# martinhoT/Footsies-Gym

Hardware: AMD Instinct MI355X
Metric: env-steps/sec (whole node) at 65 536 envs; bit-exact vs Unity ref (higher is better)
Workload: dtype int32+f32 (reward f64); 1 GPU; C3: 65536 arenas/GPU, self-play random actions, P2 external, auto-reset same-step; envs_per_gpu=65536, global_envs=65536, mode=fused, ticks_per_launch=1000, trajectory=packed records (fs_step_n_packed), parallelism=arena-shard x1, action_rows=2665, action_rows_needed=2665, action_rows_repeat=False

## Files before the change

footsies_gym_amd/csrc/fs_kernels.hip:

```cpp
#include <hip/hip_runtime.h>

#include <cstdio>

#include "fs_internal.h"
#include "fs_tables.h"
#include "fs_policy.h"

#pragma clang fp contract(off)

namespace fsk {

constexpr int NONE = 31;
constexpr uint32_t IN_LEFT = 1, IN_RIGHT = 2, IN_ATTACK = 4;

__shared__ Tables sT;
__shared__ ParserTable sParser;

constexpr int kBlock = 256;

template <bool G>
__device__ __forceinline__ const Tables& tabs() {
  if constexpr (G) return kTables;
  else return sT;
}
constexpr int kTabLds = 0, kTabGlobal = 1;


typedef float F2 __attribute__((ext_vector_type(2)));
__device__ __forceinline__ F2 splat(float v) { return F2{v, v}; }

struct Fighter {
  float x;
  uint32_t hist;
  int act, frame, stun, vital, guard, hits, buf, rsv, hold;
  uint32_t in_back, prox, won;
  int rec;
  float px, ux0, ux1, hx0, hx1;
  float pw, phw;
  uint32_t flip;
  float y;
  float py, uy0, uy1, hy0, hy1;
};

constexpr uint32_t kHdrRecCountMask = 0x7fff;
constexpr int kHdrRec1 = 15, kHdrRec2 = 18, kHdrAct1 = 21, kHdrAct2 = 24;
constexpr int kHdrPending = 27, kHdrHasTerm = 28, kHdrP2Bot = 29;
struct Header {
  uint32_t rec_count;
  uint32_t rec[2], act[2];
  uint32_t pending, has_term;
  uint32_t p2bot;
};
__device__ __forceinline__ Header unpack_header(uint32_t h) {
  return Header{h & kHdrRecCountMask, {(h >> kHdrRec1) & 7, (h >> kHdrRec2) & 7},
                {(h >> kHdrAct1) & 7, (h >> kHdrAct2) & 7}, (h >> kHdrPending) & 1, (h >> kHdrHasTerm) & 1,
                (h >> kHdrP2Bot) & 1};
}
__device__ __forceinline__ uint32_t pack_header(const Header& H) {
  return H.rec_count | (H.rec[0] << kHdrRec1) | (H.rec[1] << kHdrRec2) | (H.act[0] << kHdrAct1) |
         (H.act[1] << kHdrAct2) | (H.pending << kHdrPending) | (H.has_term << kHdrHasTerm) | (H.p2bot << kHdrP2Bot);
}

struct Arena {
  Fighter f0, f1;
  int frame_count;
  Header h;
  double cum;
  uint4 rng;
  uint2 bw[2];
// ... 93 lines not shown
  x &= 0x55555555u;
  x = (x | (x >> 1)) & 0x33333333u;
  x = (x | (x >> 2)) & 0x0F0F0F0Fu;
  x = (x | (x >> 4)) & 0x00FF00FFu;
  x = (x | (x >> 8)) & 0x0000FFFFu;
  return x;
}
__device__ __forceinline__ uint32_t spread_even(uint32_t x) {
  x &= 0x0000FFFFu;
  x = (x | (x << 8)) & 0x00FF00FFu;
  x = (x | (x << 4)) & 0x0F0F0F0Fu;
  x = (x | (x << 2)) & 0x33333333u;
  x = (x | (x << 1)) & 0x55555555u;
  return x;
}
__device__ __forceinline__ uint32_t split_hist(uint32_t raw, int k) {
  const uint32_t rel = k == 0 ? raw : (((raw & 0x55555555u) << 1) | ((raw >> 1) & 0x55555555u));
  return compact_even(rel) | (compact_even(rel >> 1) << 16);
}
__device__ __forceinline__ uint32_t raw_hist(uint32_t h, int k) {
  const uint32_t b = spread_even(h), f = spread_even(h >> 16);
  return k == 0 ? (b | (f << 1)) : (f | (b << 1));
}

constexpr uint32_t kRelLut0 = 0xE4E4u, kRelLut1 = 0xD8D8u;

__device__ __forceinline__ InputEval update_input(Fighter& f, uint32_t in, uint32_t rlut) {
  const uint32_t old_hist = f.hist;
  const int old_hold = f.hold;
  const uint32_t r0 = __builtin_amdgcn_ubfe(rlut, in << 1, 2);
  f.hist = ((old_hist << 1) & 0xFFFEFFFEu) | (r0 & 1) | ((r0 & 2) << 15);
  f.hold = (in & IN_ATTACK) ? min(old_hold + 1, 63) : 0;
  InputEval e;
  e.held = r0;
  const uint32_t atk_now = (in >> 2) & 1u;
  const uint32_t held_long = ((uint32_t)(old_hold - (kSpecialHoldFrame - 1)) >> 31) ^ 1u;
  const uint32_t was_up = (uint32_t)(old_hold - 1) >> 31;
  e.atk = (held_long & ~atk_now & 1u) | ((atk_now & was_up) << 1);
  const uint32_t B = old_hist & 0xFFFFu, F = old_hist >> 16, E = B | F;
  const uint32_t win = (1u << (kDashAllowFrame - 1)) - 1u;
  const uint32_t j = (uint32_t)__builtin_ctz((E & win) | (1u << (kDashAllowFrame - 1)));
  const uint32_t neutral = min((~E >> (j + 1)) & win, 1u);
  const uint32_t isF = ((F & win) >> j) & 1u, isB = ((B & win) >> j) & 1u;
  const uint32_t fd = isF & ~isB & neutral & (r0 >> 1) & ~F;
  const uint32_t bd = isB & ~isF & neutral & r0 & ~B;
  e.dash = (fd & 1u) | ((bd & 1u) << 1);
  return e;
}

#ifndef FS_PARSER_TABLE
#define FS_PARSER_TABLE 1
#endif
constexpr bool kParserTable = FS_PARSER_TABLE != 0;
constexpr uint32_t kRelLut4_0 = 0x64206420u, kRelLut4_1 = 0x62406240u;
__device__ __forceinline__ uint32_t pairs_hist(uint32_t h) { return spread_even(h) | (spread_even(h >> 16) << 1); }
__device__ __forceinline__ uint32_t unpair_hist(uint32_t p) { return compact_even(p) | (compact_even(p >> 1) << 16); }
__device__ __forceinline__ uint32_t parser_state_row(uint32_t h) {
  constexpr uint32_t w = kDashAllowFrame - 1, cap = kParserRunCap;
  static_assert(cap == w + 1 && 2 * w <= 16 && kParserStates == w * 3 * cap + 1, "the automaton of gen_tables.py");
  const uint32_t B = h & 0xFFFFu, F = h >> 16, E = B | F;
  const uint32_t j = (uint32_t)__builtin_ctz((E & ((1u << w) - 1u)) | (1u << w));
  const uint32_t kind = ((B >> j) & 1u) | (((F >> j) & 1u) << 1);
  const uint32_t run = min((uint32_t)__builtin_ctz(~(E >> j)), cap);
  const uint32_t s = j == w ? 0u : ((run - 1u) * w + j) * 3u + kind;
  return s << 3;
}
__device__ __forceinline__ uint32_t parser_read_row(uint32_t row, uint32_t rowb, uint32_t rlut4) {
  const uint32_t r0x2 = __builtin_amdgcn_ubfe(rlut4, rowb << 2, 3);
  return *reinterpret_cast<const uint16_t*>(reinterpret_cast<const char*>(&sParser.next[0][0]) + (row | r0x2));
}
__device__ __forceinline__ InputEval take_input(Fighter& f, uint32_t in, uint32_t pe) {
  const int old_hold = f.hold;
  InputEval e;
  e.held = (pe >> 1) & 3u;
  e.dh = pe & 0x1Eu;
  e.dash = (pe >> 3) & 3u;
  f.hist = (f.hist << 2) | e.held;
  f.hold = (in & IN_ATTACK) ? min(old_hold + 1, 63) : 0;
  const uint32_t atk_now = (in >> 2) & 1u;
  const uint32_t held_long = ((uint32_t)(old_hold - (kSpecialHoldFrame - 1)) >> 31) ^ 1u;
  const uint32_t was_up = (uint32_t)(old_hold - 1) >> 31;
  e.atk = (held_long & ~atk_now & 1u) | ((atk_now & was_up) << 1);
  return e;
}

__device__ __forceinline__ void set_action(Fighter& f, int a) {
  f.act = a;
  f.frame = 0;
  f.hits = 0;
  f.buf = NONE;
  f.rsv = NONE;
}

typedef uint32_t AInfo __attribute__((ext_vector_type(4)));
template <bool G>
__device__ __forceinline__ AInfo action_info(int a) { return reinterpret_cast<const AInfo*>(tabs<G>().action)[a]; }
__device__ __forceinline__ AInfo stand_info() {
  AInfo i;
  i.x = kStandInfo[0];
  i.y = kStandInfo[1];
  i.z = kStandInfo[2];
  i.w = kStandInfo[3];
  return i;
}
__device__ __forceinline__ int ai_frame_count(AInfo i) { return (int)(int16_t)(i.x & 0xffffu); }
__device__ __forceinline__ int ai_loop_from(AInfo i) { return (int)(int16_t)(i.x >> 16); }
__device__ __forceinline__ bool ai_always_cancel(AInfo i) { return (i.y & 0xffu) != 0; }
__device__ __forceinline__ int ai_cancel_lo(AInfo i) { return (int)((i.y >> 16) & 0xffu); }
__device__ __forceinline__ int ai_cancel_hi(AInfo i) { return (int)(i.y >> 24); }
__device__ __forceinline__ uint32_t ai_cancel_mask(AInfo i) { return i.z; }
static_assert(sizeof(ActionInfo) == 16, "ActionInfo must be 16 bytes");

__device__ __forceinline__ void increment_action_frame(Fighter& f, AInfo ai) {
  const bool stunned = f.stun > 0;
  f.stun -= stunned ? 1 : 0;
  const int next = f.frame + 1;
  const int loop_from = ai_loop_from(ai);
  const int looped = (next >= ai_frame_count(ai) && loop_from >= 0) ? loop_from : next;
  f.frame = stunned ? f.frame : looped;
}

template <bool INV = false>
__device__ __forceinline__ uint32_t request_sel_cls(const Fighter& f, const InputEval& e, uint32_t cls, bool& keep) {
  const int rsv = f.rsv, buf = f.buf;
  const bool has_rsv = rsv != NONE;
  const bool won = f.won != 0;
  const bool early = (f.stun <= 0) & (has_rsv | ((buf != NONE) & (kCanCancelOnWhiff | (f.hits > 0))));
  const int a0 = has_rsv ? rsv : buf;
  const uint32_t in8 = ((9u * cls + 3u * e.atk + e.dash) << 3) | (e.held << 1) | (uint32_t)f.prox;
  const uint32_t idx = ((uint32_t)f.act << 8) | (in8 ^ (uint32_t)f.act);
  if constexpr (INV) {
    keep = early;
    if constexpr (kParserTable) {
      const uint32_t t8 = (((9u * cls + 3u * e.atk) << 3) + e.dh) | (uint32_t)f.prox;
      return early ? (uint32_t)(kReqEarly + a0) : (((uint32_t)f.act << 8) | (t8 ^ (uint32_t)f.act));
    }
    return early ? (uint32_t)(kReqEarly + a0) : idx;
  }
  keep = early | won;
  return won ? (uint32_t)kReqWin + 3u * (uint32_t)f.act + cls : (early ? (uint32_t)(kReqEarly + a0) : idx);
}
__device__ __forceinline__ uint32_t request_cls(const Fighter& f, AInfo ai) {
  const bool ended = f.frame >= ai_frame_count(ai);
  const bool inwin = (f.frame >= ai_cancel_lo(ai)) & (f.frame <= ai_cancel_hi(ai));
  return ended ? 2u : (inwin ? 1u : 0u);
}
__device__ __forceinline__ uint32_t request_sel(const Fighter& f, const InputEval& e, AInfo ai, bool& keep) {
  return request_sel_cls(f, e, request_cls(f, ai), keep);
}
__device__ __forceinline__ bool apply_request(Fighter& f, uint32_t q, bool keep, const InputEval& e, uint32_t* rec) {
  const bool set = ((q >> 11) & 1u) != 0;
  const bool bset = ((q >> 10) & 1u) != 0;
  f.act = set ? (int)(q & 31u) : f.act;
  f.buf = set ? NONE : (bset ? (int)((q >> 5) & 31u) : f.buf);
  f.frame = set ? 0 : f.frame;
  f.hits = set ? 0 : f.hits;
  f.rsv = set ? NONE : f.rsv;
  f.in_back = keep ? f.in_back : (e.held & 1u);
  f.prox = keep ? f.prox : 0u;
  *rec = (q >> 12) & 255u;
  return set;
}
template <bool G>
__device__ __forceinline__ bool update_action_request(Fighter& f, const InputEval& e, AInfo ai, uint32_t* rec) {
  bool keep;
  const uint32_t sel = request_sel(f, e, ai, keep);
  return apply_request(f, tabs<G>().req_table[sel], keep, e, rec);
}

template <int FM>
__device__ __forceinline__ void update_movement(Fighter& f, float v) {
  float nx;
  if constexpr (FM == FS_FLOAT_DOUBLE) nx = (float)__dadd_rn((double)f.x, __dmul_rn((double)v, (double)kDt));
  else nx = __fadd_rn(f.x, __fmul_rn(v, kDt));
  f.x = (f.stun <= 0 && v != 0.0f) ? nx : f.x;
}

typedef float F4 __attribute__((ext_vector_type(4)));
typedef uint32_t U4 __attribute__((ext_vector_type(4)));
struct RecGeo {
  F4 push;
  F4 hurt;
  F4 hit;
};
template <bool G>
__device__ __forceinline__ RecGeo frame_rec(uint32_t k, uint32_t rec) {
  const Tables& T = tabs<G>();
// ... 213 lines not shown
  switch (b) {
    case 0: return r <= 3 ? AP_NONE : AP_DELAY_SPECIAL;
    case 1: return r <= 1 ? AP_NONE : r <= 3 ? AP_ONE_HIT : AP_DELAY_SPECIAL;
    case 2: return r == 0 ? AP_NONE : r == 1 ? AP_ONE_HIT : AP_TWO_HIT;
    case 3: return r <= 1 ? AP_ONE_HIT : r <= 3 ? AP_TWO_HIT : r == 4 ? AP_IMMEDIATE_SPECIAL : AP_DELAY_SPECIAL;
    default: return r == 0 ? AP_ONE_HIT : AP_TWO_HIT;
  }
}
__device__ __forceinline__ bool attack_forced(uint32_t b, uint32_t opp) {
  constexpr uint32_t kAny = (1u << A_DAMAGE) | (1u << A_GUARD_BREAK) | (1u << A_N_SPECIAL) | (1u << A_B_SPECIAL);
  constexpr uint32_t kMid = (1u << A_N_ATTACK) | (1u << A_B_ATTACK);
  return (((b == 1 ? kAny | kMid : kAny) >> opp) & 1u) != 0;
}

struct alignas(16) BotDraw {
  uint32_t map;
  uint32_t magic;
  uint32_t n;
  uint32_t c16;
};
struct alignas(16) BotTables {
  BotDraw draw[2][5];
  uint32_t codes[2][8][8];
  uint8_t len[2][8];
};
constexpr BotDraw make_draw(uint32_t n, uint32_t map) {
  return BotDraw{map, (uint32_t)(((1u << 23) + n - 1) / n), n, 65536u % n};
}
constexpr BotTables make_bot_tables() {
  BotTables t{};
  for (int b = 0; b < 5; b++) {
    uint32_t mm = 0, ma = 0;
    for (uint32_t r = 0; r < move_draw_n(b); r++) mm |= move_draw_plan(b, r) << (4 * r);
    for (uint32_t r = 0; r < attack_draw_n(b); r++) ma |= attack_draw_plan(b, r) << (4 * r);
    t.draw[1][b] = make_draw(move_draw_n(b), mm);
    t.draw[0][b] = make_draw(attack_draw_n(b), ma);
  }
  for (uint32_t p = 0; p < 7; p++) {
    t.len[1][p] = (uint8_t)move_plan_len(p);
    for (uint32_t i = 0; i < move_plan_len(p); i++) t.codes[1][p][i >> 4] |= move_plan_input(p, i) << (2 * (i & 15));
  }
  for (uint32_t p = 0; p < 5; p++) {
    t.len[0][p] = (uint8_t)attack_plan_len(p);
    for (uint32_t i = 0; i < attack_plan_len(p); i++)
      t.codes[0][p][i >> 4] |= (uint32_t)((i < attack_plan_hold(p)) | ((p == AP_TWO_HIT) & (i == 4))) << (2 * (i & 15));
  }
  return t;
}
static_assert(move_plan_len(MP_FAR1) <= 8 * 16 && attack_plan_len(AP_DELAY_SPECIAL) <= 8 * 16,
              "plans fit eight code words");
__constant__ const BotTables kBot = make_bot_tables();
__shared__ BotTables sBot;
static_assert(sizeof(Tables) + sizeof(BotTables) <= 40 * 1024, "the staged tables: at most 40 KB per block");
static_assert(sizeof(Tables) + sizeof(ParserTable) <= 40 * 1024, "(no kernel stages both: see step_body)");
template <bool G>
__device__ __forceinline__ const BotTables& bots() {
  if constexpr (G) return kBot;
  else return sBot;
}

typedef __attribute__((address_space(1))) void* GlobalPtr;
typedef __attribute__((address_space(3))) void* LdsPtr;
template <int BYTES>
__device__ __forceinline__ void lds_dma_copy(void* dst, const void* src) {
  static_assert(BYTES % 16 == 0, "16-byte pieces");
  constexpr int kChunks = BYTES / 16, kPieces = (kChunks + 63) / 64;
  const int wave = threadIdx.x >> 6, lane = threadIdx.x & 63;
  for (int j = wave; j < kPieces; j += kBlock / 64) {
    const int c = j * 64 + lane;
    if (c < kChunks)
      __builtin_amdgcn_global_load_lds((GlobalPtr)(reinterpret_cast<const char*>(src) + c * 16),
                                       (LdsPtr)(reinterpret_cast<char*>(dst) + j * 1024), 16, 0, 0);
  }
}
template <bool BOTS = true, bool PARSER = false>
__device__ __forceinline__ void stage_tables() {
  static_assert(!(BOTS && PARSER), "the bot kernels have no specialised loop");
  lds_dma_copy<sizeof(Tables)>(&sT, &kTables);
  if constexpr (BOTS) lds_dma_copy<sizeof(BotTables)>(&sBot, &kBot);
  if constexpr (PARSER) lds_dma_copy<sizeof(ParserTable)>(&sParser, &kParser);
  __syncthreads();
}

__device__ __forceinline__ uint32_t draw_mod(uint32_t x, const BotDraw& d) {
  const uint32_t v = __umul24(x >> 16, d.c16) + (x & 0xFFFFu);
  const uint64_t prod = (uint64_t)(v & 0xFFFFFFu) * (uint64_t)(d.magic & 0xFFFFFFu);
  const uint32_t q = (uint32_t)(prod >> 23);
  return v - __umul24(d.n, q);
}

struct Bot {
  uint4 rng;
  uint32_t plan, idx;
  uint32_t prev_opp;
  float prev_dist;
};

template <int FM>
__device__ __forceinline__ float bot_distance(float x1, float x2) {
  return fabsf(fsub<FM>(x2, x1));
}

__device__ __forceinline__ uint32_t xpair(uint32_t v);
struct BotPre {
  uint32_t code_word;
  BotDraw w;
  uint32_t len;
};
__device__ __forceinline__ uint32_t bot_bucket(float d) {
  return d > 4.0f ? 0u : d > 3.0f ? 1u : d > 2.5f ? 2u : d > 2.0f ? 3u : 4u;
}
template <bool G>
__device__ __forceinline__ BotPre bot_prefetch(const Bot& b, uint32_t q) {
  const uint32_t p = b.plan != 0 ? b.plan - 1 : 0u;
  BotPre r;
  r.code_word = bots<G>().codes[q][p][b.idx >> 4];
  r.w = bots<G>().draw[q][bot_bucket(b.prev_dist)];
  r.len = bots<G>().len[q][p];
  return r;
}

template <bool G>
__device__ __forceinline__ uint32_t bot_next_input(Bot& b, uint32_t q, float dist, uint32_t opp_act, const BotPre& pre) {
  const float d = b.prev_dist;
  const uint32_t opp = b.prev_opp;
  b.prev_dist = dist;
  b.prev_opp = opp_act;
  const uint32_t bucket = bot_bucket(d);
  const bool busy = b.plan != 0;
  const uint32_t i = b.idx;
  const uint32_t code = (pre.code_word >> (2 * (i & 15))) & 3u;
  const uint32_t mine = busy ? (q ? code : code << 2) : 0u;
  const bool o_busy = xpair((uint32_t)busy) != 0;
// ... 68 lines not shown
  }
  if (b.aplan != 0) {
    const uint32_t p = b.aplan - 1, i = b.aidx;
    in |= ((bots<G>().codes[0][p][i >> 4] >> (2 * (i & 15))) & 1u) << 2;
    b.aidx = i + 1;
    if (b.aidx == bots<G>().len[0][p]) b.aplan = 0;
  } else if (attack_forced(bucket, opp)) {
    b.aplan = AP_TWO_HIT + 1;
    b.aidx = 0;
  } else {
    const BotDraw w = bots<G>().draw[0][bucket];
    b.aplan = ((w.map >> (4 * draw_mod(rng_next(rng), w))) & 15u) + 1;
    b.aidx = 0;
  }
  return in;
}

__device__ __forceinline__ void bot_full_reset(FullBot& b, float dist, uint32_t opp_act) {
  b.mplan = b.midx = b.aplan = b.aidx = 0;
  b.prev_dist = dist;
  b.prev_opp = opp_act;
  b.ready = true;
}

__device__ __forceinline__ uint32_t xpair(uint32_t v) {
  return (uint32_t)__builtin_amdgcn_mov_dpp((int)v, 0xB1 , 0xF, 0xF, true);
}
__device__ __forceinline__ int xpair(int v) { return (int)xpair((uint32_t)v); }
__device__ __forceinline__ float xpair(float v) { return __uint_as_float(xpair(__float_as_uint(v))); }
__device__ __forceinline__ uint32_t xp1(uint32_t v) {
  return (uint32_t)__builtin_amdgcn_mov_dpp((int)v, 0xA0 , 0xF, 0xF, true);
}
__device__ __forceinline__ uint32_t xp2(uint32_t v) {
  return (uint32_t)__builtin_amdgcn_mov_dpp((int)v, 0xF5 , 0xF, 0xF, true);
}
__device__ __forceinline__ float xp1(float v) { return __uint_as_float(xp1(__float_as_uint(v))); }
__device__ __forceinline__ float xp2(float v) { return __uint_as_float(xp2(__float_as_uint(v))); }

struct Lane {
  Fighter f;
  uint32_t k;
  int frame_count;
  uint32_t rec_count;
  uint32_t pending, has_term;
  double cum;
  uint32_t rec;
  uint32_t act;
  uint32_t bin;
  uint32_t p2bot;
  AInfo ai;
  uint32_t te;
  uint32_t pe;
  uint32_t ps;
  Bot bot;
  FullBot fb;
  uint4 rng;
};

template <int V>
__device__ __forceinline__ void load_lane(Lane& L, const DevState& s, int a, uint32_t k) {
  const int l = 2 * a + (int)k;
  L.k = k;
  L.f.x = reinterpret_cast<const float*>(s.pos)[l];
  L.f.hist = reinterpret_cast<const uint32_t*>(s.hist)[l];
  const uint2 w = reinterpret_cast<const uint2*>(s.fpk)[l];
  const int2 aw = s.aw[a];
  L.cum = s.cum[a];
  unpack_fighter(L.f, w.x, w.y);
  const uint32_t h = (uint32_t)aw.y;
  L.frame_count = aw.x;
  L.rec_count = h & kHdrRecCountMask;
  L.rec = (h >> (k ? kHdrRec2 : kHdrRec1)) & 7;
  L.act = (h >> (k ? kHdrAct2 : kHdrAct1)) & 7;
  L.pending = (h >> kHdrPending) & 1;
  L.has_term = (h >> kHdrHasTerm) & 1;
  L.p2bot = (h >> kHdrP2Bot) & 1;
  L.bin = 0;
  if constexpr (V == FS_P2_BOT) {
    L.bot.rng = s.rng[a];
    const uint2 b = s.bot[a];
    L.bot.plan = k ? ((b.x >> kBotMoveQueue) & 7) : ((b.x >> kBotAtkQueue) & 7);
    L.bot.idx = k ? ((b.x >> kBotMoveIdx) & 127) : ((b.x >> kBotAtkIdx) & 127);
    L.bot.prev_opp = (b.x >> kBotPrevOpp) & 31;
    L.bot.prev_dist = __uint_as_float(b.y);
    L.bin = (b.x >> kBotInput) & 7;
  } else if constexpr (V == kActors) {
    L.rng = s.rng[a];
    L.fb = unpack_bot(k ? s.bot[a] : s.bot1[a], L.bin);
  }
}

template <int V>
__device__ __forceinline__ void store_lane(const Lane& L, const DevState& s, int a) {
  const int l = 2 * a + (int)L.k;
  const uint64_t w = pack_fighter(L.f);
  reinterpret_cast<float*>(s.pos)[l] = L.f.x;
  reinterpret_cast<uint32_t*>(s.hist)[l] = L.f.hist;
  reinterpret_cast<uint2*>(s.fpk)[l] = make_uint2((uint32_t)w, (uint32_t)(w >> 32));
  const uint32_t other = xpair(L.rec | (L.act << 3));
  if (L.k == 0) {
    const uint32_t p2bot = V == FS_P2_BOT ? 1u : V == kActors ? (uint32_t)L.p2bot : 0u;
    const uint32_t h = L.rec_count | (L.rec << kHdrRec1) | ((other & 7) << kHdrRec2) | (L.act << kHdrAct1) |
                       ((other >> 3) << kHdrAct2) | ((uint32_t)L.pending << kHdrPending) |
                       ((uint32_t)L.has_term << kHdrHasTerm) | (p2bot << kHdrP2Bot);
    s.aw[a] = make_int2(L.frame_count, (int)h);
    s.cum[a] = L.cum;
// ... 277 lines not shown
  const PkRec v = packed_record(L, 0u);
  const uint32_t ox = xpair(v.x), oz = xpair(v.z);
  RecQ q;
  if (L.k == 0) {
    q.x = __builtin_amdgcn_perm(ox, v.x, 0x05010400u);
    q.y = __builtin_amdgcn_perm(ox, v.x, 0x07030602u);
    q.z = terminated;
    q.w = v.y;
  } else {
    q.x = v.y;
    q.y = oz;
    q.z = v.z;
    q.w = (uint32_t)L.frame_count;
  }
  char* b = reinterpret_cast<char*>(rec) + 40u * r;
  *reinterpret_cast<RecQ*>(b + 16u * L.k) = q;
  if (L.k == 0) {
    const uint64_t rw = (uint64_t)__double_as_longlong(reward);
    *reinterpret_cast<uint2*>(b + 32u) = make_uint2((uint32_t)rw, (uint32_t)(rw >> 32));
  }
}

__device__ __forceinline__ uint64_t splitmix64(uint64_t x) {
  x += 0x9E3779B97F4A7C15ull;
  x = (x ^ (x >> 30)) * 0xBF58476D1CE4E5B9ull;
  x = (x ^ (x >> 27)) * 0x94D049BB133111EBull;
  return x ^ (x >> 31);
}
__device__ __forceinline__ uint32_t hash_action(uint64_t seed, uint64_t env, uint64_t t, uint32_t player) {
  return (uint32_t)(splitmix64(seed ^ (env * 0x9E3779B97F4A7C15ull) ^ ((t << 1) | player)) & 7u);
}


__device__ __forceinline__ uint32_t row_load(const uint8_t* p) {
  uint32_t v;
  asm volatile("global_load_ubyte %0, %1, off" : "=v"(v) : "v"(p) : "memory");
  return v;
}
template <int WAIT>
__device__ __forceinline__ void settle_w(uint32_t& next) {
  if constexpr (WAIT < 0) {
    asm volatile("" : "+v"(next));
  } else {
    uint32_t ready;
    asm volatile("s_waitcnt vmcnt(%2)\n\tv_mov_b32 %0, %1" : "=v"(ready) : "v"(next), "n"(WAIT) : "memory");
    next = ready;
  }
}

constexpr int kPrioSliceShift = 9;
__device__ __forceinline__ uint32_t prio_group() {
  return __builtin_amdgcn_s_getreg(4  | (31 << 11)) & 1u;
}
__device__ __forceinline__ void prio_slice(uint32_t grp) {
  const uint32_t now = (uint32_t)__builtin_amdgcn_s_memrealtime() ^ (grp << kPrioSliceShift);
  asm volatile("s_bitcmp1_b32 %0, %1\n\ts_cbranch_scc0 .Lprio_lo%=\n\ts_setprio 1\n\ts_branch .Lprio_end%=\n"
               ".Lprio_lo%=:\n\ts_setprio 0\n.Lprio_end%=:" :: "s"(now), "n"(kPrioSliceShift) : "scc");
}

constexpr int kLmGeneric = 0;
#ifndef FS_ROW_DEPTH2
#define FS_ROW_DEPTH2 4
#endif
constexpr int kLmFast = 1;
constexpr int kLmFastPrio = 2;
__device__ __forceinline__ bool in_fast_set(const Fighter& f) {
  constexpr uint32_t kOut = (1u << A_DEAD) | (1u << A_WIN);
  static_assert(A_DEAD < 31 && A_WIN < 31, "");
  const uint32_t named = (1u << f.act) | (1u << f.buf) | (1u << f.rsv);
  return (f.won == 0) & ((named & kOut) == 0) & (f.frame < kTickFrames) & (f.vital == 1);
}

template <bool G, bool FLAGS = true>
__device__ __forceinline__ void opaque_burst_results(Lane& L) {
  if constexpr (FLAGS)
    asm volatile("" : "+v"(L.f.x), "+v"(L.f.act), "+v"(L.f.frame), "+v"(L.f.vital), "+v"(L.f.guard), "+v"(L.f.hits),
                 "+v"(L.f.buf), "+v"(L.f.rsv), "+v"(L.f.hold), "+v"(L.f.won), "+v"(L.f.hist));
  else
    asm volatile("" : "+v"(L.f.x), "+v"(L.f.act), "+v"(L.f.frame), "+v"(L.f.vital), "+v"(L.f.guard), "+v"(L.f.hits),
                 "+v"(L.f.buf), "+v"(L.f.rsv), "+v"(L.f.hold), "+v"(L.f.hist));
  if constexpr (G) asm volatile("" : "+v"(L.ai));
  else asm volatile("" : "+v"(L.te));
  if constexpr (FLAGS)
    asm volatile("" : "+v"(L.cum), "+v"(L.pending), "+v"(L.has_term), "+v"(L.frame_count), "+v"(L.rec_count));
  else asm volatile("" : "+v"(L.cum), "+v"(L.frame_count), "+v"(L.rec_count));
  if constexpr (!FLAGS && kParserTable) asm volatile("" : "+v"(L.ps));
}

struct Pre {
  InputEval e;
  uint32_t q;
  int rec_cont;
  uint32_t keep;
};
template <int P2>
__device__ __forceinline__ uint32_t tick_input(const Lane& L, uint32_t a_own) {
  static_assert(P2 != kActors, "(the per-arena actors take env_step's own path)");
  if (L.k == 0 || P2 == FS_P2_EXTERNAL) return a_own;
  return P2 == FS_P2_BOT ? L.bin : 0u;
}
template <int P2>
__device__ __forceinline__ uint32_t parser_rlut(uint32_t k) {
  static_assert(P2 == FS_P2_EXTERNAL || P2 == FS_P2_NOOP, "the kernels with a specialised loop");
  return k ? (P2 == FS_P2_NOOP ? 0u : kRelLut4_1) : kRelLut4_0;
}

template <int P2>
__device__ __forceinline__ void parser_enter(Lane& L, uint32_t row) {
  L.ps = parser_state_row(L.f.hist);
  L.pe = parser_read_row(L.ps, row, parser_rlut<P2>(L.k));
  L.f.hist = pairs_hist(L.f.hist);
}
__device__ __forceinline__ void parser_leave(Lane& L) { L.f.hist = unpair_hist(L.f.hist); }

template <bool INV = false>
__device__ __forceinline__ void prepare_request(Lane& L, uint32_t in, Pre& pre) {
  if constexpr (INV && kParserTable) {
    pre.e = take_input(L.f, in, L.pe);
    L.ps = L.pe >> 5;
  } else pre.e = update_input(L.f, in, L.k ? kRelLut1 : kRelLut0);
  const uint32_t cls = tick_begin(L.f, L.te, &pre.rec_cont);
  bool keep;
  const uint32_t sel = request_sel_cls<INV>(L.f, pre.e, cls, keep);
  pre.keep = keep;
  pre.q = sT.req_table[sel];
}

enum StepKind { kOneTick, kRows, kHashed, kPolicy };
constexpr unsigned kGeom = 1, kPacked = 2, kPrefetch = 4;
constexpr int kWaitTracked = -1;
template <int FM_, int P2_, StepKind KIND_, unsigned OPTS_ = 0, int LM_ = kLmGeneric, int WAIT_ = kWaitTracked,
          int DEPTH_ = 2>
struct TickCfg {
  static constexpr int FM = FM_, P2 = P2_, LM = LM_, WAIT = WAIT_;
  static constexpr int DEPTH = DEPTH_;
  static_assert(DEPTH >= 2 && DEPTH <= 4 && (DEPTH == 2 || LM_ != kLmGeneric), "row ring depth: 2..4, the fast loops only");
  static constexpr StepKind KIND = KIND_;
  static constexpr unsigned OPTS = OPTS_;
  static constexpr bool GEOM = (OPTS & kGeom) != 0, PK = (OPTS & kPacked) != 0, PF = (OPTS & kPrefetch) != 0;
  static constexpr int TP = KIND == kOneTick ? kTabGlobal : kTabLds;
  static_assert(!PK || KIND == kRows, "packed trajectories: the fused row loop only");
  static_assert(!PF || (KIND == kRows && !GEOM && P2 != kActors), "request prefetch: the standard row loop");
  static_assert(LM == kLmGeneric || KIND == kRows, "launch modes: the fused row loop only");
};
#define FS_TICK(C) C::FM, C::P2, C::WAIT, C::TP, C::GEOM, C::PK, C::PF, C::LM

template <int FM, int P2, int WAIT, int TP, bool GEOM, bool PK, bool PF, int LM>
__device__ __forceinline__ void env_step(Lane& L, uint32_t a_own, const StepParams& p, uint32_t r, uint32_t& next,
                                         const Pre& pre = Pre{}, bool use_pre = false) {
  constexpr bool BOT = P2 == FS_P2_BOT;
  constexpr bool G = TP == kTabGlobal;
  const DevOutputs& o = p.out;
  const uint32_t k = L.k;
  const Actors ac{p.p1_bot != 0, p.p2_resets != 0, p.p2_noop != 0};
  constexpr bool FAST = LM != kLmGeneric;
  if (!FAST && L.pending) {
    reset_burst<FM, P2, G>(L, true, ac);
    if constexpr (GEOM) {
      L.f.y = 0.0f;
      L.f.flip = 0;
    }
    L.pending = false;
    L.has_term = false;
    L.cum = 0.0;
    if constexpr (G) L.ai = stand_info();
    else L.te = tick_entry(L.f);
    settle_w<WAIT>(next);
    if constexpr (PK) {
      write_packed(L, o.pk_lanes, r, k == 0 ? (uint32_t)L.frame_count : 0u);
      st_off(o.reward, 8 * r, 0.0);
    } else {
      write_main(L, o, r);
      st_off(o.reward, 8 * r, 0.0);
      st_off(o.terminated, r, (uint8_t)0);
      st_off(o.truncated, r, (uint8_t)0);
      if constexpr (G) {
        if (p.rec) write_record(L, p.rec, r, 0u, 0.0);
      }
    }
    opaque_burst_results<G>(L);
    return;
  }
  uint32_t in;
  if constexpr (P2 == kActors) {
    const bool mybot = k == 0 ? ac.p1_bot : L.p2bot;
    const bool idle = k == 1 && ac.p2_noop;
    L.act = (!mybot && !idle) ? a_own : L.act;
    in = mybot ? L.bin : (idle ? 0u : L.act);
  } else {
    if (k == 0 || P2 == FS_P2_EXTERNAL) L.act = a_own;
    in = (BOT && k == 1) ? L.bin : ((P2 == FS_P2_NOOP && k == 1) ? 0u : L.act);
  }
  const int guard_before = L.f.guard;
  BotPre bpre;
  if constexpr (BOT) bpre = bot_prefetch<G>(L.bot, k);
  L.frame_count++;
  if constexpr (FAST) {
    const bool recs = L.rec_count < kMaxRecording;
    L.rec = recs ? in : L.rec;
    L.rec_count += recs ? 1u : 0u;
  } else if (L.rec_count < kMaxRecording) {
    L.rec = in;
    L.rec_count++;
  }
  const uint32_t face = GEOM ? k ^ L.f.flip : k;
  InputEval e;
  int rec_cont;
  uint32_t rec_set;
  bool set;
  if (PF && use_pre) {
    e = pre.e;
    rec_cont = pre.rec_cont;
    set = apply_request(L.f, pre.q, pre.keep != 0, e, &rec_set);
  } else {
    if constexpr (FAST && kParserTable) {
      e = take_input(L.f, in, L.pe);
      L.ps = L.pe >> 5;
    } else e = update_input(L.f, in, face ? kRelLut1 : kRelLut0);
    if constexpr (G) {
      const AInfo ai = L.ai;
      increment_action_frame(L.f, ai);
      rec_cont = frame_record<G>(L.f);
      set = update_action_request<G>(L.f, e, ai, &rec_set);
    } else {
      const uint32_t cls = tick_begin(L.f, L.te, &rec_cont);
      bool keep;
      const uint32_t sel = request_sel_cls<FAST>(L.f, e, cls, keep);
      set = apply_request(L.f, sT.req_table[sel], keep, e, &rec_set);
    }
  }
  L.f.rec = set ? (int)rec_set : rec_cont;
  const RecGeo R = frame_rec<G>(face, (uint32_t)L.f.rec);
  const uint32_t o_rec = (uint32_t)xpair(L.f.rec);
  const uint32_t o_hits = (uint32_t)xpair(L.f.hits);
  static_assert(kNumFrameRecs <= 64, "ybits rows are 64 records wide");
  const uint32_t ym = tabs<G>().ybits[(o_rec << 6) | (uint32_t)L.f.rec];
  const U4 res = reinterpret_cast<const U4*>(tabs<G>().resolve)[__umul24(o_hits, (uint32_t)kNumFrameRecs) + o_rec];
  update_movement<FM>(L.f, R.push.z);
  update_boxes<FM>(L.f, R);
  RecY Y;
  if constexpr (GEOM) {
    Y = rec_y((uint32_t)L.f.rec);
    update_boxes_y<FM>(L.f, Y);
  }
  const float o_hw0 = xpair(R.hit.z), o_hw1 = xpair(R.hit.w);
  push_character_vs_character<FM, GEOM>(L.f, k, GEOM ? Y.a.y : 0.0f);
  push_character_vs_background<FM, GEOM>(L.f);
  asm volatile("" ::"v"(R.push), "v"(R.hurt), "v"(o_hw0), "v"(o_hw1), "v"(res), "v"(ym));
  uint32_t ym_t = ym;
  if constexpr (GEOM) {
    const float o_hy0 = xpair(L.f.hy0), o_hy1 = xpair(L.f.hy1), o_hh0 = xpair(Y.b.w), o_hh1 = xpair(Y.c.y);
    const float hymax0 = fadd<FM>(o_hy0, o_hh0), hymax1 = fadd<FM>(o_hy1, o_hh1);
    const float uymax0 = fadd<FM>(L.f.uy0, Y.a.w), uymax1 = fadd<FM>(L.f.uy1, Y.b.y);
    auto ov = [](float uy, float uymax, float hy, float hymax) { return (uint32_t)((uymax >= hy) & (uy <= hymax)); };
    ym_t = ov(L.f.uy0, uymax0, o_hy0, hymax0) | (ov(L.f.uy1, uymax1, o_hy0, hymax0) << 1) |
           (ov(L.f.uy0, uymax0, o_hy1, hymax1) << 2) | (ov(L.f.uy1, uymax1, o_hy1, hymax1) << 3);
  }
  const uint32_t tab = collision_lookup<FM>(L.f, R.hurt, o_hw0, o_hw1, res, ym_t);
  bool wave_hit = true;
  const uint32_t prox_before = L.f.prox;
  if constexpr (FAST) {
    wave_hit = wave_has_hit(tab);
    proximity_latch(L.f, tab);
    asm volatile("" : "+v"(L.f.prox));
  }
  if (__builtin_expect(wave_hit, !FAST)) {
    if constexpr (FAST) L.f.prox = prox_before;
    collision_resolve(L.f, k, tab);
  }
  if constexpr (!G) L.te = next_tick_entry<PF, FAST>(L.f);
  if constexpr (FAST) settle_w<WAIT>(next);
  bool over = false;
  double reward = 0.0;
  if (__builtin_expect(wave_hit, !FAST)) {
    const uint32_t my_fl = ((uint32_t)(L.f.vital - 1) >> 31) | (((uint32_t)(L.f.guard - guard_before) >> 31) << 1);
    const uint32_t o_fl = xpair(my_fl);
    const uint32_t any_fl = my_fl | o_fl;
    over = (any_fl & 1u) != 0;
    if (FAST || p.dense_reward) {
      if (any_fl != 0) {
        const uint32_t fl1 = k == 0 ? my_fl : o_fl, fl2 = k == 0 ? o_fl : my_fl;
        if (fl1 & 2u) reward -= 0.3;
        if (fl2 & 2u) reward += 0.3;
        L.cum += reward;
        if (over) reward += (double)((fl2 & 1u) ? 1 : -1) - L.cum;
      }
    } else {
      const uint32_t fl2 = k == 0 ? o_fl : my_fl;
      reward = over ? ((fl2 & 1u) ? 1.0 : -1.0) : 0.0;
    }
    if constexpr (!FAST) settle_w<WAIT>(next);
    if (over) {
      L.f.hist = 0;
      L.f.hold = 0;
      if (FAST || p.autoreset_mode == FS_AUTORESET_SAME_STEP) {
        if constexpr (PK) write_packed(L, o.pk_final, r, k == 0 ? (uint32_t)L.frame_count : 0u);
        else write_final(L, o, r);
        reset_burst<FM, P2, G, FAST && kParserTable>(L, true, ac);
        if constexpr (GEOM) {
          L.f.y = 0.0f;
          L.f.flip = 0;
        }
        L.cum = 0.0;
        if constexpr (!FAST) L.has_term = false;
        if constexpr (G) L.ai = stand_info();
        else L.te = tick_entry(L.f);
        if constexpr (FAST && kParserTable) L.ps = L.f.hist << 3;
        if constexpr (FAST) opaque_burst_results<G, false>(L);
      } else {
        L.pending = true;
        L.has_term = true;
      }
    } else {
      if constexpr (BOT) {
        const float x1 = xp1(L.f.x), x2 = xp2(L.f.x);
        const uint32_t p1_act = xp1((uint32_t)L.f.act);
        const uint32_t bi = bot_next_input<G>(L.bot, k, bot_distance<FM>(x1, x2), p1_act, bpre);
        L.bin = k == 1 ? bi : L.bin;
      } else if constexpr (P2 == kActors) {
        const float x1 = xp1(L.f.x), x2 = xp2(L.f.x);
        const uint32_t p1_act = xp1((uint32_t)L.f.act), p2_act = xp2((uint32_t)L.f.act);
        actors_request<G>(L, ac, bot_distance<FM>(x1, x2), p1_act, p2_act);
      }
      if constexpr (!FAST) L.has_term = false;
    }
  }
  if constexpr (FAST && kParserTable) L.pe = parser_read_row(L.ps, next, parser_rlut<P2>(k));
  if constexpr (PK) {
    write_packed<!FAST>(L, o.pk_lanes, r, k == 0 ? (uint32_t)L.frame_count : (over ? 1u : 0u));
    st_off(o.reward, 8 * r, reward);
  } else {
    write_main<!FAST>(L, o, r);
    st_off(o.reward, 8 * r, reward);
    st_off(o.terminated, r, (uint8_t)(over ? 1 : 0));
    st_off(o.truncated, r, (uint8_t)0);
    if constexpr (G) {
      if (p.rec) write_record(L, p.rec, r, over ? 1u : 0u, reward);
    }
  }
  if constexpr (!G) asm volatile("" ::"v"(L.te));
}

__device__ __forceinline__ void policy_features(const Lane& L, uint32_t& d0, uint32_t& d1) {
  int a = L.f.act;
  if (a == A_DEAD || a == A_WIN) a = A_STAND;
  const int mf = (a == A_STAND || a == A_FORWARD || a == A_BACKWARD) ? 0 : L.f.frame;
  d0 = pack_bf16x2((float)L.f.guard * (1.0f / 3.0f), (float)a * (1.0f / 16.0f));
  d1 = pack_bf16x2((float)mf * (1.0f / 55.0f), L.f.x * (1.0f / 4.6f));
}

template <bool PK>
constexpr int row_wait(int depth) {
  constexpr int kRowWait = PK ? 3 : 11;
  constexpr int kRowOps = PK ? 3 : 11;
  return kRowWait + kRowOps * (depth - 2);
}

template <class C>
__device__ __forceinline__ void row_ring(Lane& L, const StepParams& p, bool reads, const uint8_t* own, uint32_t row_mul,
                                         int a, uint32_t row0, uint32_t row1, uint32_t row2, uint32_t row3) {
  constexpr int P2 = C::P2, LM = C::LM, D = C::DEPTH;
  constexpr bool PF = C::PF;
  static_assert(LM != kLmGeneric && D > 2 && row_wait<C::PK>(D) <= 63, "the fast loops' ring; vmcnt has six bits");
  using Tick = TickCfg<C::FM, P2, kRows, C::OPTS, LM, row_wait<C::PK>(D), D>;
  L.f.won = 0;
  const int n = p.n_steps, last = n - 1;
  const uint32_t row_step = (uint32_t)p.out_stride_steps * (uint32_t)p.n_envs;
  const uint32_t grp = prio_group();
  uint32_t fl[4] = {row0, row1, row2, row3};
  uint32_t rd = row0;
  Pre pre{};
  bool have = false;
  if constexpr (kParserTable) parser_enter<P2>(L, row0);
  auto issue = [&](int t) -> uint32_t { return row_load(own + (uint32_t)min(t, last) * row_mul + (uint32_t)a); };
  auto tick = [&](int t, auto J, bool use_pre) {
    constexpr int j = decltype(J)::value, jn = (j + 1) % D;
    fl[j] = issue(t + D);
    if constexpr (LM == kLmFastPrio) prio_slice(grp);
    uint32_t next = fl[jn];
    env_step<FS_TICK(Tick)>(L, reads ? rd & 7u : 0u, p, (uint32_t)t * row_step + (uint32_t)a, next, pre, use_pre);
    rd = next;
  };
  auto prepare = [&] {
    if constexpr (PF) prepare_request<true>(L, tick_input<P2>(L, reads ? rd & 7u : 0u), pre);
  };
  int t = 0;
  for (; t + D <= n; t += D) {
    tick(t, std::integral_constant<int, 0>{}, have);
    prepare();
    have = PF;
    tick(t + 1, std::integral_constant<int, 1>{}, PF);
    prepare();
    tick(t + 2, std::integral_constant<int, 2>{}, PF);
    if constexpr (D > 3) {
      prepare();
      tick(t + 3, std::integral_constant<int, 3 % D>{}, PF);
    }
    if constexpr (PF) {
      if (t + D <= last) prepare();
    }
  }
  if (t < n) {
    tick(t, std::integral_constant<int, 0>{}, have);
    if (t + 1 < n) {
      prepare();
      tick(t + 1, std::integral_constant<int, 1>{}, PF);
      if constexpr (D > 3) {
        if (t + 2 < n) {
          prepare();
          tick(t + 2, std::integral_constant<int, 2>{}, PF);
        }
      }
    }
  }
  asm volatile("s_waitcnt vmcnt(0)" ::"v"(fl[0]), "v"(fl[1]), "v"(fl[2]), "v"(fl[3]) : "memory");
  if constexpr (kParserTable) parser_leave(L);
  L.pending = L.has_term = 0;
}

template <class C>
__device__ __forceinline__ void row_loop(Lane& L, const StepParams& p, bool reads, const uint8_t* own, uint32_t row_mul,
                                         int a, uint32_t row0, uint32_t row1) {
  static_assert(C::DEPTH == 2, "deeper: row_ring");
  constexpr int P2 = C::P2, LM = C::LM;
  constexpr bool PF = C::PF;
  using Tick = TickCfg<C::FM, P2, kRows, C::OPTS, LM, row_wait<C::PK>(2)>;
  constexpr bool PRIO = LM == kLmFastPrio;
  if constexpr (LM != kLmGeneric) L.f.won = 0;
  const int last = p.n_steps - 1;
  const uint32_t row_step = (uint32_t)p.out_stride_steps * (uint32_t)p.n_envs;
  uint32_t a_fl = row0, b_fl = row1, a_rd = row0, b_rd = row1;
  const uint32_t grp = prio_group();
  if constexpr (LM != kLmGeneric && kParserTable) parser_enter<P2>(L, row0);
  auto slice = [&] {
    if constexpr (PRIO) prio_slice(grp);
    else if constexpr (LM == kLmGeneric) {
      if (p.prio) prio_slice(grp);
    }
  };
  Pre pre{};
  bool have = false;
  auto issue = [&](int t) -> uint32_t { return row_load(own + (uint32_t)min(t, last) * row_mul + (uint32_t)a); };
  int t = 0;
  for (; t < last; t += 2) {
    a_fl = issue(t + 2);
    slice();
    env_step<FS_TICK(Tick)>(L, reads ? a_rd & 7u : 0u, p, (uint32_t)t * row_step + (uint32_t)a, b_fl, pre, have);
    b_rd = b_fl;
    if constexpr (PF) {
      prepare_request<LM != kLmGeneric>(L, tick_input<P2>(L, reads ? b_rd & 7u : 0u), pre);
      have = true;
    }
    b_fl = issue(t + 3);
    slice();
    env_step<FS_TICK(Tick)>(L, reads ? b_rd & 7u : 0u, p, (uint32_t)(t + 1) * row_step + (uint32_t)a, a_fl, pre, PF);
    a_rd = a_fl;
    if constexpr (PF) {
      if (t + 2 <= last) prepare_request<LM != kLmGeneric>(L, tick_input<P2>(L, reads ? a_rd & 7u : 0u), pre);
    }
  }
  if (t == last) {
    a_fl = issue(t + 2);
    uint32_t b_last = b_fl;
// ... 827 lines not shown
```

footsies_gym_amd/csrc/fs_tables.h:

```cpp
#pragma once
#include <stdint.h>
namespace fsk {
constexpr int kNumActions = 17;
constexpr int kNumRows = 892;
constexpr int kNumRects = 23;
constexpr int kNumVels = 16;
constexpr int kNumHurtSets = 11;
constexpr int kNumHitSets = 10;
constexpr int kNumCancelMasks = 2;
constexpr int A_STAND = 0;
constexpr int A_FORWARD = 1;
constexpr int A_BACKWARD = 2;
constexpr int A_DASH_FORWARD = 3;
constexpr int A_DASH_BACKWARD = 4;
constexpr int A_N_ATTACK = 5;
constexpr int A_B_ATTACK = 6;
constexpr int A_N_SPECIAL = 7;
constexpr int A_B_SPECIAL = 8;
constexpr int A_DAMAGE = 9;
constexpr int A_GUARD_M = 10;
constexpr int A_GUARD_STAND = 11;
constexpr int A_GUARD_CROUCH = 12;
constexpr int A_GUARD_BREAK = 13;
constexpr int A_GUARD_PROXIMITY = 14;
// ... 1259 lines not shown
  {0x0000, 0x0112, 0x0204, 0x0316},
  {0x0000, 0x0102, 0x020c, 0x030e},
  {0x0000, 0x0102, 0x0204, 0x0306},
  {0xac00, 0xc102, 0xc204, 0xc306},
  {0xad00, 0xc102, 0xc204, 0xc306},
  {0xae00, 0xc102, 0xc204, 0xc306},
  {0xaf00, 0x0112, 0x0204, 0x0316},
  {0xb000, 0x0102, 0x020c, 0x030e},
  {0xb100, 0x0102, 0x0204, 0x0306},
  {0xb200, 0x0112, 0x0204, 0x0316},
  {0xb300, 0x0102, 0x020c, 0x030e},
  {0xb400, 0x0102, 0x0204, 0x0306},
  {0xb500, 0x0112, 0x0204, 0x0316},
  {0xb600, 0x0102, 0x020c, 0x030e},
  {0xb700, 0x0102, 0x0204, 0x0306},
  {0xb800, 0x0112, 0x0204, 0x0316},
  {0xb900, 0x0102, 0x020c, 0x030e},
  {0xba00, 0x0102, 0x0204, 0x0306},
  {0xbb00, 0x0112, 0x0204, 0x0316},
  {0xbc00, 0x0102, 0x020c, 0x030e},
  {0xbd00, 0x0102, 0x0204, 0x0306},
  {0xbe00, 0x0112, 0x0204, 0x0316},
  {0xbf00, 0x0102, 0x020c, 0x030e},
  {0xc000, 0x0102, 0x0204, 0x0306},
  {0x0000, 0x0112, 0x0204, 0x0316},
  {0x0000, 0x0102, 0x020c, 0x030e},
  {0x0000, 0x0102, 0x0204, 0x0306},
  {0xc400, 0xc102, 0xc204, 0xc306},
  {0xc500, 0xc102, 0xc204, 0xc306},
  {0xc600, 0xc102, 0xc204, 0xc306},
  {0xc700, 0x0102, 0x0204, 0x0306},
  {0xc800, 0x0102, 0x0204, 0x0306},
  {0xc900, 0x0102, 0x0204, 0x0306},
  {0xca00, 0x0102, 0x0204, 0x0306},
  {0xcb00, 0x0102, 0x0204, 0x0306},
  {0xcc00, 0x0102, 0x0204, 0x0306},
  {0xcd00, 0x0102, 0x0204, 0x0306},
  {0xce00, 0x0102, 0x0204, 0x0306},
  {0xcf00, 0x0102, 0x0204, 0x0306},
  {0xd000, 0x0102, 0x0204, 0x0306},
  {0xd100, 0x0102, 0x0204, 0x0306},
  {0xd200, 0x0102, 0x0204, 0x0306},
  {0xd300, 0x0102, 0x0204, 0x0306},
  {0xd400, 0x0102, 0x0204, 0x0306},
  {0xd500, 0x0102, 0x0204, 0x0306},
  {0xd600, 0x0102, 0x0204, 0x0306},
  {0xd700, 0x0102, 0x0204, 0x0306},
  {0xd800, 0x0102, 0x0204, 0x0306},
  {0x0000, 0x0102, 0x0204, 0x0306},
  {0x0000, 0x0102, 0x0204, 0x0306},
  {0x0000, 0x0102, 0x0204, 0x0306},
  {0x0000, 0x0000, 0x0000, 0x0000},
}};
__constant__ const int16_t kActionId[kNumActions] = {0, 1, 2, 10, 11, 100, 105, 110, 115, 200, 301, 305, 306, 310, 350, 500, 510};
}
```

Measured before the change: 86.05 billion env-steps/s.

## Add LDS hold-counter transition table and per-turn priority clock sampling

Replaces the per-tick arithmetic that updates the attack-hold counter and derives the attack event with a 64x2 lookup table staged in LDS. The next tick's entry is prefetched alongside the parser row. The priority slicing now reads the realtime clock once per unrolled turn instead of every tick. The terminated flag is also routed through an opaque register with a branch hint. The aim is to shorten the serial per-tick instruction chain, at the cost of an extra LDS load per tick, more LDS footprint and a held register.

```diff
diff --git a/footsies_gym_amd/csrc/fs_kernels.hip b/footsies_gym_amd/csrc/fs_kernels.hip
--- a/footsies_gym_amd/csrc/fs_kernels.hip
+++ b/footsies_gym_amd/csrc/fs_kernels.hip
@@ -15,6 +15,7 @@
 
 __shared__ Tables sT;
 __shared__ ParserTable sParser;
+__shared__ HoldTable sHold;
 
 constexpr int kBlock = 256;
 
@@ -214,6 +215,14 @@
 #define FS_PARSER_TABLE 1
 #endif
 constexpr bool kParserTable = FS_PARSER_TABLE != 0;
+#ifndef FS_REQ_SELECT
+#define FS_REQ_SELECT 1
+#endif
+constexpr bool kReqSelect = FS_REQ_SELECT != 0;
+#ifndef FS_HOLD_TABLE
+#define FS_HOLD_TABLE 1
+#endif
+constexpr bool kHoldTable = FS_HOLD_TABLE != 0 && kParserTable;
 constexpr uint32_t kRelLut4_0 = 0x64206420u, kRelLut4_1 = 0x62406240u;
 __device__ __forceinline__ uint32_t pairs_hist(uint32_t h) { return spread_even(h) | (spread_even(h >> 16) << 1); }
 __device__ __forceinline__ uint32_t unpair_hist(uint32_t p) { return compact_even(p) | (compact_even(p >> 1) << 16); }
@@ -231,13 +240,22 @@
   const uint32_t r0x2 = __builtin_amdgcn_ubfe(rlut4, rowb << 2, 3);
   return *reinterpret_cast<const uint16_t*>(reinterpret_cast<const char*>(&sParser.next[0][0]) + (row | r0x2));
 }
-__device__ __forceinline__ InputEval take_input(Fighter& f, uint32_t in, uint32_t pe) {
+__device__ __forceinline__ uint32_t hold_read_row(uint32_t hold, uint32_t rowb, uint32_t amask) {
+  static_assert(IN_ATTACK == sizeof(uint32_t) && sizeof(sHold.next[0]) == 8, "the attack bit is the entry's byte offset");
+  return *reinterpret_cast<const uint32_t*>(reinterpret_cast<const char*>(&sHold.next[0][0]) + ((hold << 3) | (rowb & amask)));
+}
+__device__ __forceinline__ InputEval take_input(Fighter& f, uint32_t in, uint32_t pe, uint32_t he) {
   const int old_hold = f.hold;
   InputEval e;
   e.held = (pe >> 1) & 3u;
   e.dh = pe & 0x1Eu;
   e.dash = (pe >> 3) & 3u;
   f.hist = (f.hist << 2) | e.held;
+  if constexpr (kHoldTable) {
+    f.hold = (int)(he & 0xFFFFu);
+    e.atk = he >> 16;
+    return e;
+  }
   f.hold = (in & IN_ATTACK) ? min(old_hold + 1, 63) : 0;
   const uint32_t atk_now = (in >> 2) & 1u;
   const uint32_t held_long = ((uint32_t)(old_hold - (kSpecialHoldFrame - 1)) >> 31) ^ 1u;
@@ -294,7 +312,11 @@
   if constexpr (INV) {
     keep = early;
     if constexpr (kParserTable) {
-      const uint32_t t8 = (((9u * cls + 3u * e.atk) << 3) + e.dh) | (uint32_t)f.prox;
+      const uint32_t t8 = ((kHoldTable ? 72u * cls + e.atk : (9u * cls + 3u * e.atk) << 3) + e.dh) | (uint32_t)f.prox;
+      if constexpr (kReqSelect) {
+        const uint32_t ix = ((uint32_t)f.act << 8) | (t8 ^ (uint32_t)f.act), ea = (uint32_t)(kReqEarly + a0);
+        return early ? ea : ix;
+      }
       return early ? (uint32_t)(kReqEarly + a0) : (((uint32_t)f.act << 8) | (t8 ^ (uint32_t)f.act));
     }
     return early ? (uint32_t)(kReqEarly + a0) : idx;
@@ -614,7 +636,7 @@
 __constant__ const BotTables kBot = make_bot_tables();
 __shared__ BotTables sBot;
 static_assert(sizeof(Tables) + sizeof(BotTables) <= 40 * 1024, "the staged tables: at most 40 KB per block");
-static_assert(sizeof(Tables) + sizeof(ParserTable) <= 40 * 1024, "(no kernel stages both: see step_body)");
+static_assert(sizeof(Tables) + sizeof(ParserTable) + sizeof(HoldTable) <= 40 * 1024, "(no kernel stages both: see step_body)");
 template <bool G>
 __device__ __forceinline__ const BotTables& bots() {
   if constexpr (G) return kBot;
@@ -641,6 +663,7 @@
   lds_dma_copy<sizeof(Tables)>(&sT, &kTables);
   if constexpr (BOTS) lds_dma_copy<sizeof(BotTables)>(&sBot, &kBot);
   if constexpr (PARSER) lds_dma_copy<sizeof(ParserTable)>(&sParser, &kParser);
+  if constexpr (PARSER && kHoldTable) lds_dma_copy<sizeof(HoldTable)>(&sHold, &kHold);
   __syncthreads();
 }
 
@@ -815,6 +838,7 @@
   uint32_t te;
   uint32_t pe;
   uint32_t ps;
+  uint32_t he;
   Bot bot;
   FullBot fb;
   uint4 rng;
@@ -1198,11 +1222,17 @@
 __device__ __forceinline__ uint32_t prio_group() {
   return __builtin_amdgcn_s_getreg(4  | (31 << 11)) & 1u;
 }
-__device__ __forceinline__ void prio_slice(uint32_t grp) {
-  const uint32_t now = (uint32_t)__builtin_amdgcn_s_memrealtime() ^ (grp << kPrioSliceShift);
+__device__ __forceinline__ uint32_t prio_clock() { return (uint32_t)__builtin_amdgcn_s_memrealtime(); }
+__device__ __forceinline__ void prio_apply(uint32_t clock, uint32_t grp) {
+  const uint32_t now = clock ^ (grp << kPrioSliceShift);
   asm volatile("s_bitcmp1_b32 %0, %1\n\ts_cbranch_scc0 .Lprio_lo%=\n\ts_setprio 1\n\ts_branch .Lprio_end%=\n"
                ".Lprio_lo%=:\n\ts_setprio 0\n.Lprio_end%=:" :: "s"(now), "n"(kPrioSliceShift) : "scc");
 }
+__device__ __forceinline__ void prio_slice(uint32_t grp) { prio_apply(prio_clock(), grp); }
+#ifndef FS_PRIO_PER_TURN
+#define FS_PRIO_PER_TURN 1
+#endif
+constexpr bool kPrioPerTurn = FS_PRIO_PER_TURN != 0;
 
 constexpr int kLmGeneric = 0;
 #ifndef FS_ROW_DEPTH2
@@ -1250,11 +1280,17 @@
   static_assert(P2 == FS_P2_EXTERNAL || P2 == FS_P2_NOOP, "the kernels with a specialised loop");
   return k ? (P2 == FS_P2_NOOP ? 0u : kRelLut4_1) : kRelLut4_0;
 }
+template <int P2>
+__device__ __forceinline__ uint32_t hold_amask(uint32_t k) {
+  static_assert(P2 == FS_P2_EXTERNAL || P2 == FS_P2_NOOP, "the kernels with a specialised loop");
+  return (k && P2 == FS_P2_NOOP) ? 0u : IN_ATTACK;
+}
 
 template <int P2>
 __device__ __forceinline__ void parser_enter(Lane& L, uint32_t row) {
   L.ps = parser_state_row(L.f.hist);
   L.pe = parser_read_row(L.ps, row, parser_rlut<P2>(L.k));
+  if constexpr (kHoldTable) L.he = hold_read_row((uint32_t)L.f.hold, row, hold_amask<P2>(L.k));
   L.f.hist = pairs_hist(L.f.hist);
 }
 __device__ __forceinline__ void parser_leave(Lane& L) { L.f.hist = unpair_hist(L.f.hist); }
@@ -1262,7 +1298,7 @@
 template <bool INV = false>
 __device__ __forceinline__ void prepare_request(Lane& L, uint32_t in, Pre& pre) {
   if constexpr (INV && kParserTable) {
-    pre.e = take_input(L.f, in, L.pe);
+    pre.e = take_input(L.f, in, L.pe, L.he);
     L.ps = L.pe >> 5;
   } else pre.e = update_input(L.f, in, L.k ? kRelLut1 : kRelLut0);
   const uint32_t cls = tick_begin(L.f, L.te, &pre.rec_cont);
@@ -1360,7 +1396,7 @@
     set = apply_request(L.f, pre.q, pre.keep != 0, e, &rec_set);
   } else {
     if constexpr (FAST && kParserTable) {
-      e = take_input(L.f, in, L.pe);
+      e = take_input(L.f, in, L.pe, L.he);
       L.ps = L.pe >> 5;
     } else e = update_input(L.f, in, face ? kRelLut1 : kRelLut0);
     if constexpr (G) {
@@ -1418,6 +1454,7 @@
   if constexpr (FAST) settle_w<WAIT>(next);
   bool over = false;
   double reward = 0.0;
+  uint32_t over_w = 0;
   if (__builtin_expect(wave_hit, !FAST)) {
     const uint32_t my_fl = ((uint32_t)(L.f.vital - 1) >> 31) | (((uint32_t)(L.f.guard - guard_before) >> 31) << 1);
     const uint32_t o_fl = xpair(my_fl);
@@ -1436,7 +1473,7 @@
       reward = over ? ((fl2 & 1u) ? 1.0 : -1.0) : 0.0;
     }
     if constexpr (!FAST) settle_w<WAIT>(next);
-    if (over) {
+    if ((FAST && kReqSelect) ? __builtin_expect(over, 0) : over) {
       L.f.hist = 0;
       L.f.hold = 0;
       if (FAST || p.autoreset_mode == FS_AUTORESET_SAME_STEP) {
@@ -1470,15 +1507,20 @@
       }
       if constexpr (!FAST) L.has_term = false;
     }
+    if constexpr (FAST && kReqSelect && !PK) {
+      over_w = over ? 1u : 0u;
+      asm volatile("" : "+v"(over_w));
+    }
   }
   if constexpr (FAST && kParserTable) L.pe = parser_read_row(L.ps, next, parser_rlut<P2>(k));
+  if constexpr (FAST && kHoldTable) L.he = hold_read_row((uint32_t)L.f.hold, next, hold_amask<P2>(k));
   if constexpr (PK) {
     write_packed<!FAST>(L, o.pk_lanes, r, k == 0 ? (uint32_t)L.frame_count : (over ? 1u : 0u));
     st_off(o.reward, 8 * r, reward);
   } else {
     write_main<!FAST>(L, o, r);
     st_off(o.reward, 8 * r, reward);
-    st_off(o.terminated, r, (uint8_t)(over ? 1 : 0));
+    st_off(o.terminated, r, (FAST && kReqSelect) ? (uint8_t)over_w : (uint8_t)(over ? 1 : 0));
     st_off(o.truncated, r, (uint8_t)0);
     if constexpr (G) {
       if (p.rec) write_record(L, p.rec, r, over ? 1u : 0u, reward);
@@ -1519,42 +1561,51 @@
   bool have = false;
   if constexpr (kParserTable) parser_enter<P2>(L, row0);
   auto issue = [&](int t) -> uint32_t { return row_load(own + (uint32_t)min(t, last) * row_mul + (uint32_t)a); };
-  auto tick = [&](int t, auto J, bool use_pre) {
+  constexpr bool kTurnClock = LM == kLmFastPrio && kPrioPerTurn;
+  uint32_t clock = 0;
+  if constexpr (kTurnClock) clock = prio_clock();
+  auto tick = [&](int t, auto J, bool use_pre, auto TURN) {
     constexpr int j = decltype(J)::value, jn = (j + 1) % D;
+    constexpr bool turn = decltype(TURN)::value;
     fl[j] = issue(t + D);
-    if constexpr (LM == kLmFastPrio) prio_slice(grp);
+    if constexpr (kTurnClock) {
+      if constexpr (turn && j == 0) prio_apply(clock, grp);
+    } else if constexpr (LM == kLmFastPrio) prio_slice(grp);
     uint32_t next = fl[jn];
     env_step<FS_TICK(Tick)>(L, reads ? rd & 7u : 0u, p, (uint32_t)t * row_step + (uint32_t)a, next, pre, use_pre);
     rd = next;
+    if constexpr (kTurnClock && turn && j == D - 1) clock = prio_clock();
   };
+  constexpr std::true_type in_turn{};
+  constexpr std::false_type in_rest{};
   auto prepare = [&] {
     if constexpr (PF) prepare_request<true>(L, tick_input<P2>(L, reads ? rd & 7u : 0u), pre);
   };
   int t = 0;
   for (; t + D <= n; t += D) {
-    tick(t, std::integral_constant<int, 0>{}, have);
+    tick(t, std::integral_constant<int, 0>{}, have, in_turn);
     prepare();
     have = PF;
-    tick(t + 1, std::integral_constant<int, 1>{}, PF);
+    tick(t + 1, std::integral_constant<int, 1>{}, PF, in_turn);
     prepare();
-    tick(t + 2, std::integral_constant<int, 2>{}, PF);
+    tick(t + 2, std::integral_constant<int, 2>{}, PF, in_turn);
     if constexpr (D > 3) {
       prepare();
-      tick(t + 3, std::integral_constant<int, 3 % D>{}, PF);
+      tick(t + 3, std::integral_constant<int, 3 % D>{}, PF, in_turn);
     }
     if constexpr (PF) {
       if (t + D <= last) prepare();
     }
   }
   if (t < n) {
-    tick(t, std::integral_constant<int, 0>{}, have);
+    tick(t, std::integral_constant<int, 0>{}, have, in_rest);
     if (t + 1 < n) {
       prepare();
-      tick(t + 1, std::integral_constant<int, 1>{}, PF);
+      tick(t + 1, std::integral_constant<int, 1>{}, PF, in_rest);
       if constexpr (D > 3) {
         if (t + 2 < n) {
           prepare();
-          tick(t + 2, std::integral_constant<int, 2>{}, PF);
+          tick(t + 2, std::integral_constant<int, 2>{}, PF, in_rest);
         }
       }
     }
diff --git a/footsies_gym_amd/csrc/fs_tables.h b/footsies_gym_amd/csrc/fs_tables.h
--- a/footsies_gym_amd/csrc/fs_tables.h
+++ b/footsies_gym_amd/csrc/fs_tables.h
@@ -1335,5 +1335,25 @@
   {0x0000, 0x0102, 0x0204, 0x0306},
   {0x0000, 0x0000, 0x0000, 0x0000},
 }};
+constexpr int kHoldCap = 63;
+struct alignas(16) HoldTable { uint32_t next[64][2]; };
+__constant__ const HoldTable kHold = {{
+  {0x000000, 0x300001}, {0x000000, 0x000002}, {0x000000, 0x000003}, {0x000000, 0x000004},
+  {0x000000, 0x000005}, {0x000000, 0x000006}, {0x000000, 0x000007}, {0x000000, 0x000008},
+  {0x000000, 0x000009}, {0x000000, 0x00000a}, {0x000000, 0x00000b}, {0x000000, 0x00000c},
+  {0x000000, 0x00000d}, {0x000000, 0x00000e}, {0x000000, 0x00000f}, {0x000000, 0x000010},
+  {0x000000, 0x000011}, {0x000000, 0x000012}, {0x000000, 0x000013}, {0x000000, 0x000014},
+  {0x000000, 0x000015}, {0x000000, 0x000016}, {0x000000, 0x000017}, {0x000000, 0x000018},
+  {0x000000, 0x000019}, {0x000000, 0x00001a}, {0x000000, 0x00001b}, {0x000000, 0x00001c},
+  {0x000000, 0x00001d}, {0x000000, 0x00001e}, {0x000000, 0x00001f}, {0x000000, 0x000020},
+  {0x000000, 0x000021}, {0x000000, 0x000022}, {0x000000, 0x000023}, {0x000000, 0x000024},
+  {0x000000, 0x000025}, {0x000000, 0x000026}, {0x000000, 0x000027}, {0x000000, 0x000028},
+  {0x000000, 0x000029}, {0x000000, 0x00002a}, {0x000000, 0x00002b}, {0x000000, 0x00002c},
+  {0x000000, 0x00002d}, {0x000000, 0x00002e}, {0x000000, 0x00002f}, {0x000000, 0x000030},
+  {0x000000, 0x000031}, {0x000000, 0x000032}, {0x000000, 0x000033}, {0x000000, 0x000034},
+  {0x000000, 0x000035}, {0x000000, 0x000036}, {0x000000, 0x000037}, {0x000000, 0x000038},
+  {0x000000, 0x000039}, {0x000000, 0x00003a}, {0x000000, 0x00003b}, {0x180000, 0x00003c},
+  {0x180000, 0x00003d}, {0x180000, 0x00003e}, {0x180000, 0x00003f}, {0x180000, 0x00003f},
+}};
 __constant__ const int16_t kActionId[kNumActions] = {0, 1, 2, 10, 11, 100, 105, 110, 115, 200, 301, 305, 306, 310, 350, 500, 510};
 }
```

Result: no change. 86.05 billion env-steps/s (-0.0%).
